# ferdean/lsa-fw

Hardware: AMD Instinct MI355X
Metric: converged eigenpairs/sec (k=20, shift-invert) (higher is better)
Workload: dtype c128

## Files before the change

### lsa-fw_amd/csrc/blas.hip

```cpp
#include "lsa_internal.h"

namespace {

constexpr int kThreads = 256;
constexpr int kColTile = 8;

template <typename T>
__device__ __forceinline__ T wave_sum(T v);
template <>
__device__ __forceinline__ double wave_sum<double>(double v) {
#pragma unroll
    for (int m = 32; m > 0; m >>= 1) v += __shfl_xor(v, m, 64);
    return v;
}
template <>
__device__ __forceinline__ cplx wave_sum<cplx>(cplx v) {
#pragma unroll
    for (int m = 32; m > 0; m >>= 1) {
        v.re += __shfl_xor(v.re, m, 64);
        v.im += __shfl_xor(v.im, m, 64);
    }
    return v;
}

// ... 775 lines not shown
                const double d = hs[j].re - s1;
                const double nu = sqrt(d < 0.0 ? 0.0 : d);
                const double inv = 1.0 / nu;
                nu_s = nu;
                c_s = s_mul(inv, s_sub(beta, s2));
            }
        }
    }
    __syncthreads();
    const double nu = nu_s, inv = 1.0 / nu;
    const cplx cc = c_s;
    if (bx == 0) {
        for (int c = threadIdx.x; c < j; c += kThreads) {
            slot[c] = first ? cplx{0.0, 0.0} : hs[c];
            if constexpr (Y) slot[lds + c] = hs[kFuseCols + c];
        }
        if (threadIdx.x == 0) {
            slot[2 * lds] = cplx{nu, 0.0};
            slot[2 * lds + 1] = cc;
        }
    }
    cplx aa = cplx{0.0, 0.0}, ab = cplx{0.0, 0.0};
    if (i < n) {
#pragma unroll
        for (int u = 0; u < 8; ++u)
            if (q + 4 * u < j) {
                if (!first) fma_acc(aa, hs[q + 4 * u], v0[u]);
                if constexpr (Y) fma_acc(ab, hs[kFuseCols + q + 4 * u], v0[u]);
            }
        for (int c = q + 32; c < j; c += 32) {
            cplx v[8];
#pragma unroll
            for (int u = 0; u < 8; ++u) v[u] = (c + 4 * u < j) ? V[i + (int64_t)(c + 4 * u) * ldv] : cplx{0.0, 0.0};
#pragma unroll
            for (int u = 0; u < 8; ++u)
                if (c + 4 * u < j) {
                    if (!first) fma_acc(aa, hs[c + 4 * u], v[u]);
                    if constexpr (Y) fma_acc(ab, hs[kFuseCols + c + 4 * u], v[u]);
                }
        }
    }
    const int l1 = (lane & 15) + 16, l2 = (lane & 15) + 32, l3 = (lane & 15) + 48;
    const cplx a1 = cplx{__shfl(aa.re, l1), __shfl(aa.im, l1)}, a2 = cplx{__shfl(aa.re, l2), __shfl(aa.im, l2)},
               a3 = cplx{__shfl(aa.re, l3), __shfl(aa.im, l3)};
    cplx b1 = cplx{0.0, 0.0}, b2 = b1, b3 = b1;
    if constexpr (Y) {
        b1 = cplx{__shfl(ab.re, l1), __shfl(ab.im, l1)};
        b2 = cplx{__shfl(ab.re, l2), __shfl(ab.im, l2)};
        b3 = cplx{__shfl(ab.re, l3), __shfl(ab.im, l3)};
    }
    double nrm = 0.0;
    if (q == 0 && i < n) {
        cplx qv = pi;
        if (!first) {
            qv = s_mul(inv, s_sub(pi, s_add(s_add(aa, a1), s_add(a2, a3))));
            V[i + (int64_t)j * ldv] = qv;
        }
        if constexpr (Y) {
            const cplx r = s_mul(inv, s_sub(s_sub(yi, s_add(s_add(ab, b1), s_add(b2, b3))), s_mul(cc, qv)));
            V[i + (int64_t)(j + 1) * ldv] = r;
            nrm = s_abs2(r);
        }
    }
    if constexpr (Y) {
        nrm = wave_sum_dpp(nrm);
        if (lane == 0) wn[wave] = nrm;
        __syncthreads();
        if (threadIdx.x == 0) nrm_part[bx] = (wn[0] + wn[1]) + (wn[2] + wn[3]);
    }
}

template <bool Y>
__global__ __launch_bounds__(kThreads) void dcgs_update_kernel(int64_t n, int j, cplx* V, int64_t ldv, const cplx* __restrict__ part, int nchunks,
                                                               int ldp, const cplx* __restrict__ y, int first, double* __restrict__ nrm_part,
                                                               cplx* __restrict__ slot, int lds, const double* __restrict__ chk_part,
                                                               double* __restrict__ chk_out) {
    dcgs_update_body<Y>((int)blockIdx.x, n, j, V, ldv, part, nchunks, ldp, y, first, nrm_part, slot, lds, chk_part, chk_out);
}

__global__ __launch_bounds__(kThreads) void dcgs_update_batch_kernel(int64_t n, int64_t ldv, int nchunks, int ldp, int lds, DcgsBatchArgs a) {
    const int z = blockIdx.z;
    dcgs_update_body<true>((int)blockIdx.x, n, a.j[z], a.V[z], ldv, a.part[z], nchunks, ldp, a.y[z], a.first[z], a.nrm_part[z], a.slot[z], lds,
                           (const double*)nullptr, (double*)nullptr);
}

__global__ __launch_bounds__(kThreads) void dcgs_norm_kernel(const double* __restrict__ nrm_part, int nparts, cplx* __restrict__ out) {
    __shared__ double smem[4];
    const double t = parts_sum(nrm_part, nparts, smem);
    if (threadIdx.x == 0) s_from(out[0], sqrt(t), 0.0);
}

__global__ __launch_bounds__(kThreads) void col_stats_kernel(int64_t n, const cplx* __restrict__ X, int64_t ldx, double* __restrict__ nrm_part,
                                                             double* __restrict__ mag_part, long long* __restrict__ idx_part) {
    __shared__ double ssum[4];
    __shared__ double smag[kThreads];
    __shared__ long long sidx[kThreads];
    const cplx* x = X + (size_t)blockIdx.y * (size_t)ldx;
    double s = 0.0, best = -1.0;
    long long bi = -1;
    const int64_t stride = (int64_t)gridDim.x * blockDim.x;
    for (int64_t i = (int64_t)blockIdx.x * blockDim.x + threadIdx.x; i < n; i += stride) {
        const double a = s_abs2(x[i]);
        s += a;
        if (a > best) {
            best = a;
            bi = i;
        }
    }
    const double tot = block_sum<double>(s, ssum);
    smag[threadIdx.x] = best;
    sidx[threadIdx.x] = bi;
    __syncthreads();
    for (int o = kThreads / 2; o > 0; o >>= 1) {
        if ((int)threadIdx.x < o) {
            const double m2 = smag[threadIdx.x + o];
            const long long i2 = sidx[threadIdx.x + o];
            if (m2 > smag[threadIdx.x] || (m2 == smag[threadIdx.x] && i2 >= 0 && (sidx[threadIdx.x] < 0 || i2 < sidx[threadIdx.x]))) {
                smag[threadIdx.x] = m2;
                sidx[threadIdx.x] = i2;
            }
        }
        __syncthreads();
    }
    if (threadIdx.x == 0) {
        const size_t at = (size_t)blockIdx.y * gridDim.x + blockIdx.x;
        nrm_part[at] = tot;
        mag_part[at] = smag[0];
        idx_part[at] = sidx[0];
    }
}

__global__ __launch_bounds__(kThreads) void col_phase_kernel(int64_t n, cplx* __restrict__ X, int64_t ldx, const double* __restrict__ nrm_part,
                                                             const double* __restrict__ mag_part, const long long* __restrict__ idx_part, int unit,
                                                             double* __restrict__ imag_part) {
    __shared__ double ssum[4];
    __shared__ double smag[kThreads];
    __shared__ long long sidx[kThreads];
    cplx* x = X + (size_t)blockIdx.y * (size_t)ldx;
    const int nb = gridDim.x;
    const size_t base = (size_t)blockIdx.y * nb;
    double s = 0.0, best = -1.0;
    long long bi = -1;
    for (int q = threadIdx.x; q < nb; q += kThreads) {
        s += nrm_part[base + q];
        const double m2 = mag_part[base + q];
        const long long i2 = idx_part[base + q];
        if (m2 > best || (m2 == best && i2 >= 0 && (bi < 0 || i2 < bi))) {
            best = m2;
            bi = i2;
        }
    }
    const double tot = block_sum<double>(s, ssum);
    smag[threadIdx.x] = best;
    sidx[threadIdx.x] = bi;
    __syncthreads();
    for (int o = kThreads / 2; o > 0; o >>= 1) {
        if ((int)threadIdx.x < o) {
            const double m2 = smag[threadIdx.x + o];
            const long long i2 = sidx[threadIdx.x + o];
            if (m2 > smag[threadIdx.x] || (m2 == smag[threadIdx.x] && i2 >= 0 && (sidx[threadIdx.x] < 0 || i2 < sidx[threadIdx.x]))) {
                smag[threadIdx.x] = m2;
                sidx[threadIdx.x] = i2;
            }
        }
        __syncthreads();
    }
// ... 451 lines not shown
    const FusedWork fw(work, 16);
    void *part1 = fw.part1, *part2 = fw.part2, *h1 = fw.h1, *h2 = fw.h2;
    double* nrm_part = fw.nrm_part;
    const dim3 dgrid(nchunks, (j + kColTile - 1) / kColTile);
    hipLaunchKernelGGL((cgs_dot_kernel<T>), dgrid, dim3(kThreads), 0, ctx->stream, n, j, rpb, (const T*)V, ldv, (const T*)y, (T*)part1, kFuseCols,
                       (const T*)nullptr, (const T*)nullptr, (double*)nullptr);
    hipLaunchKernelGGL((cgs_axpy_kernel<T>), dim3(blocks), dim3(kThreads), 0, ctx->stream, n, j, (const T*)V, ldv, (const T*)part1, nchunks, kFuseCols,
                       (const T*)y, (T*)w, (T*)h1, (double*)nullptr, (const double*)nullptr, (double*)nullptr);
    hipLaunchKernelGGL((cgs_dot_kernel<T>), dgrid, dim3(kThreads), 0, ctx->stream, n, j, rpb, (const T*)V, ldv, (const T*)w, (T*)part2, kFuseCols,
                       (const T*)nullptr, (const T*)nullptr, (double*)nullptr);
    hipLaunchKernelGGL((cgs_axpy_kernel<T>), dim3(blocks), dim3(kThreads), 0, ctx->stream, n, j, (const T*)V, ldv, (const T*)part2, nchunks, kFuseCols,
                       (const T*)w, (T*)w, (T*)h2, nrm_part, (const double*)nullptr, (double*)nullptr);
    const int tparts = k_cgs2_tail_parts(n);
    if (M->dtype == LSA_C128)
        hipLaunchKernelGGL((cgs_tail_kernel<cplx, 16>), dim3(tparts), dim3(kThreads), 0, ctx->stream, (int32_t)n, C->rp, C->ci, (const cplx*)M->val,
                           (const cplx*)C->val, (const T*)w, (const T*)y, (const double*)nrm_part, blocks, (T*)vnext, (T*)t, j, (const T*)h1, (const T*)h2,
                           (T*)hcol_dev, tail_part);
    else
        hipLaunchKernelGGL((cgs_tail_kernel<double, 16>), dim3(tparts), dim3(kThreads), 0, ctx->stream, (int32_t)n, C->rp, C->ci, (const double*)M->val,
                           (const cplx*)C->val, (const T*)w, (const T*)y, (const double*)nrm_part, blocks, (T*)vnext, (T*)t, j, (const T*)h1, (const T*)h2,
                           (T*)hcol_dev, tail_part);
    return check_launch(ctx, "cgs2_fused_tail");
}

int k_cgs2_tail_checks(lsa_ctx* ctx, int nslots, int nparts, const double* tail_parts, double* checks) {
    if (nslots <= 0) return LSA_OK;
    hipLaunchKernelGGL(cgs_tail_checks_kernel, dim3(nslots), dim3(kThreads), 0, ctx->stream, nparts, tail_parts, checks);
    return check_launch(ctx, "cgs2_tail_checks");
}

bool k_dcgs2_fits(int64_t n, int ncv) { return cgs2_fused_shape(n, ncv + 1, nullptr); }

int k_dcgs2_step(lsa_ctx* ctx, int64_t n, int j, void* V, int64_t ldv, const void* y, int first, void* slot, int lds, void* work,
                 const void* chk_b, const void* chk_z, double* chk_out) {
    int64_t rpb = 0;
    if (!cgs2_fused_shape(n, j + 1, &rpb) || j < 0 || j + 1 > lds + 1 || (first && !y))
        return lsa_set_error(ctx, LSA_ERR_ARG, "k_dcgs2_step: shape outside the fused form");
    const int nchunks = (int)((n + rpb - 1) / rpb);
    const int blocks = (int)((n + 63) / 64);
    const FusedWork fw(work, 16);
    cplx* part = (cplx*)fw.part1;
    double *chk_part = fw.chk_part, *nrm_part = fw.nrm_part;
    const dim3 dgrid(nchunks, (j + 1 + kColTile - 1) / kColTile);
    const int ldp = 2 * kFuseCols;
    if (y) {
        hipLaunchKernelGGL((dcgs_dot_kernel<true>), dgrid, dim3(kThreads), 0, ctx->stream, n, j + 1, rpb, (const cplx*)V, ldv, (const cplx*)y, part, ldp,
                           (const cplx*)chk_b, (const cplx*)chk_z, chk_out ? chk_part : (double*)nullptr);
        hipLaunchKernelGGL((dcgs_update_kernel<true>), dim3(blocks), dim3(kThreads), 0, ctx->stream, n, j, (cplx*)V, ldv, (const cplx*)part, nchunks, ldp,
                           (const cplx*)y, first, nrm_part, (cplx*)slot, lds, (const double*)chk_part, chk_out);
    } else {
        hipLaunchKernelGGL((dcgs_dot_kernel<false>), dgrid, dim3(kThreads), 0, ctx->stream, n, j + 1, rpb, (const cplx*)V, ldv, (const cplx*)nullptr, part,
                           ldp, (const cplx*)nullptr, (const cplx*)nullptr, (double*)nullptr);
        hipLaunchKernelGGL((dcgs_update_kernel<false>), dim3(blocks), dim3(kThreads), 0, ctx->stream, n, j, (cplx*)V, ldv, (const cplx*)part, nchunks, ldp,
                           (const cplx*)nullptr, 0, (double*)nullptr, (cplx*)slot, lds, (const double*)nullptr, (double*)nullptr);
    }
    return check_launch(ctx, "dcgs2_step");
}

int k_dcgs2_norm(lsa_ctx* ctx, int64_t n, void* work, void* slot, int lds) {
    double* nrm_part = FusedWork(work, 16).nrm_part;
    hipLaunchKernelGGL(dcgs_norm_kernel, dim3(1), dim3(kThreads), 0, ctx->stream, (const double*)nrm_part, (int)((n + 63) / 64),
                       (cplx*)slot + 2 * (size_t)lds + 2);
    return check_launch(ctx, "dcgs2_norm");
}

int k_dcgs2_tail(lsa_ctx* ctx, int64_t n, int j, const void* V, int64_t ldv, const void* y, void* work, const lsa_mat* M, const lsa_mat* C, void* t,
                 double* tail_part, void* slot, int lds) {
    const int blocks = (int)((n + 63) / 64);
    double* nrm_part = FusedWork(work, 16).nrm_part;
    const cplx* w = (const cplx*)V + (size_t)(j + 1) * (size_t)ldv;
    cplx* nout = (cplx*)slot + 2 * (size_t)lds + 2;
    const int tparts = k_cgs2_tail_parts(n);
    if (M->dtype == LSA_C128)
        hipLaunchKernelGGL((cgs_tail_kernel<cplx, 16, true>), dim3(tparts), dim3(kThreads), 0, ctx->stream, (int32_t)n, C->rp, C->ci, (const cplx*)M->val,
                           (const cplx*)C->val, w, (const cplx*)y, (const double*)nrm_part, blocks, (cplx*)nullptr, (cplx*)t, 0, (const cplx*)nullptr,
                           (const cplx*)nullptr, nout, tail_part);
    else
        hipLaunchKernelGGL((cgs_tail_kernel<double, 16, true>), dim3(tparts), dim3(kThreads), 0, ctx->stream, (int32_t)n, C->rp, C->ci,
                           (const double*)M->val, (const cplx*)C->val, w, (const cplx*)y, (const double*)nrm_part, blocks, (cplx*)nullptr, (cplx*)t, 0,
                           (const cplx*)nullptr, (const cplx*)nullptr, nout, tail_part);
    return check_launch(ctx, "dcgs2_tail");
}

int k_dcgs2_step_batch(lsa_ctx* ctx, int J, int64_t n, const int32_t* j, void* const* V, int64_t ldv, const void* const* y, const int32_t* first,
                       void* const* slot, int lds, void* const* work) {
    if (J < 1 || J > kKrylovGroupMax) return lsa_set_error(ctx, LSA_ERR_ARG, "k_dcgs2_step_batch: J = %d outside [1, %d]", J, kKrylovGroupMax);
    int64_t rpb = 0;
    int jmax = 0;
    DcgsBatchArgs a;
    memset(&a, 0, sizeof a);
    for (int z = 0; z < J; ++z) {
        if (j[z] < 0 || j[z] + 1 > lds + 1 || !cgs2_fused_shape(n, j[z] + 1, &rpb) || !y[z])
            return lsa_set_error(ctx, LSA_ERR_ARG, "k_dcgs2_step_batch: shape outside the fused form (problem %d)", z);
        jmax = std::max(jmax, (int)j[z]);
        const FusedWork fw(work[z], 16);
        a.V[z] = (cplx*)V[z];
        a.y[z] = (const cplx*)y[z];
        a.part[z] = (cplx*)fw.part1;
        a.slot[z] = (cplx*)slot[z];
        a.nrm_part[z] = fw.nrm_part;
        a.j[z] = j[z];
        a.first[z] = first[z];
    }
    const int nchunks = (int)((n + rpb - 1) / rpb);
    const int blocks = (int)((n + 63) / 64);
    const int ldp = 2 * kFuseCols;
    hipLaunchKernelGGL(dcgs_dot_batch_kernel, dim3(nchunks, (jmax + 1 + kColTile - 1) / kColTile, J), dim3(kThreads), 0, ctx->stream, n, rpb, ldv, ldp, a);
    hipLaunchKernelGGL(dcgs_update_batch_kernel, dim3(blocks, 1, J), dim3(kThreads), 0, ctx->stream, n, ldv, nchunks, ldp, lds, a);
    return check_launch(ctx, "dcgs2_step_batch");
}

int k_dcgs2_tail_batch(lsa_ctx* ctx, int J, int64_t n, const int32_t* j, void* const* V, int64_t ldv, const void* const* y, void* const* work,
                       const lsa_mat* const* M, const lsa_mat* const* C, void* const* t, double* const* tail_part, void* const* slot, int lds) {
    if (J < 1 || J > kKrylovGroupMax) return lsa_set_error(ctx, LSA_ERR_ARG, "k_dcgs2_tail_batch: J = %d outside [1, %d]", J, kKrylovGroupMax);
    TailBatchArgs a;
    memset(&a, 0, sizeof a);
    for (int z = 0; z < J; ++z) {
        if (M[z]->dtype != M[0]->dtype) return lsa_set_error(ctx, LSA_ERR_ARG, "k_dcgs2_tail_batch: real and complex M in one round (problem %d)", z);
        a.rp[z] = C[z]->rp;
        a.ci[z] = C[z]->ci;
        a.mval[z] = M[z]->val;
        a.cval[z] = (const cplx*)C[z]->val;
        a.w[z] = (const cplx*)V[z] + (size_t)(j[z] + 1) * (size_t)ldv;
        a.y[z] = (const cplx*)y[z];
        a.nrm_part[z] = FusedWork(work[z], 16).nrm_part;
        a.t[z] = (cplx*)t[z];
        a.hout[z] = (cplx*)slot[z] + 2 * (size_t)lds + 2;
        a.chk_part[z] = tail_part[z];
    }
    const int blocks = (int)((n + 63) / 64);
    const dim3 grid(k_cgs2_tail_parts(n), 1, J);
    if (M[0]->dtype == LSA_C128) hipLaunchKernelGGL((cgs_tail_batch_kernel<cplx, 16>), grid, dim3(kThreads), 0, ctx->stream, (int32_t)n, blocks, a);
    else hipLaunchKernelGGL((cgs_tail_batch_kernel<double, 16>), grid, dim3(kThreads), 0, ctx->stream, (int32_t)n, blocks, a);
    return check_launch(ctx, "dcgs2_tail_batch");
}
```

### lsa-fw_amd/csrc/lsa_internal.h

```cpp
#pragma once

#include <hip/hip_runtime.h>

#include <algorithm>
#include <cmath>
#include <cstdarg>
#include <cstdint>
#include <cstdio>
#include <cstdlib>
#include <cstring>
#include <memory>
#include <string>
#include <vector>

#include "../../include/lsa_hip.h"

struct cplx {
    double re, im;
};
static_assert(sizeof(cplx) == 16, "complex128 layout");

__host__ __device__ inline cplx make_cplx(double r, double i) { return cplx{r, i}; }

template <typename T>
// ... 172 lines not shown
}

#define LSA_HIP_CHECK(ctx, expr)                                                                         \
    do {                                                                                                 \
        hipError_t _e = (expr);                                                                          \
        if (_e != hipSuccess)                                                                            \
            return lsa_set_error((ctx), LSA_ERR_HIP, "%s failed: %s (%s:%d)", #expr, hipGetErrorString(_e), \
                                 __FILE__, __LINE__);                                                    \
    } while (0)

#define LSA_HIP_ALLOC(ctx, expr)                                                                                    \
    do {                                                                                                            \
        hipError_t _e = (expr);                                                                                     \
        if (_e != hipSuccess) {                                                                                     \
            (void)hipGetLastError();                                                                                \
            return lsa_set_error((ctx), _e == hipErrorOutOfMemory ? LSA_ERR_OOM : LSA_ERR_HIP, "%s failed: %s (%s:%d)", #expr, \
                                 hipGetErrorString(_e), __FILE__, __LINE__);                                        \
        }                                                                                                           \
    } while (0)

#define LSA_CHECK(expr)            \
    do {                           \
        int _rc = (expr);          \
        if (_rc != LSA_OK) return _rc; \
    } while (0)

template <typename F>
int lsa_time_runs(lsa_ctx* ctx, bool warm, int iters, double* avg_ms, F&& run) {
    if (warm) LSA_CHECK(run());
    LSA_HIP_CHECK(ctx, hipEventRecord(ctx->ev0, ctx->stream));
    for (int i = 0; i < iters; ++i) LSA_CHECK(run());
    LSA_HIP_CHECK(ctx, hipEventRecord(ctx->ev1, ctx->stream));
    LSA_HIP_CHECK(ctx, hipEventSynchronize(ctx->ev1));
    float ms = 0.f;
    LSA_HIP_CHECK(ctx, hipEventElapsedTime(&ms, ctx->ev0, ctx->ev1));
    *avg_ms = (double)ms / iters;
    return LSA_OK;
}

constexpr int kKrylovGroupMax = 16;


int k_spmv(lsa_ctx* ctx, const lsa_mat* A, int xdtype, const void* x, void* y);
int k_spmv_transpose(lsa_ctx* ctx, const lsa_mat* A, int conj, int xdtype, const void* x, void* y);
int k_transpose_index(lsa_ctx* ctx, const lsa_mat* A, const TransposeIndex** out);
int k_spmv_transpose_batch(lsa_ctx* ctx, int32_t J, const lsa_mat* const* mats, int conj, int xdtype, const void* const* xs, void* const* ys);
int k_spmv_batch(lsa_ctx* ctx, int32_t J, const lsa_mat* const* mats, int xdtype, const void* const* xs, void* const* ys);
void spmv_share_extras(const lsa_mat* from, lsa_mat* to);

int k_spmm(lsa_ctx* ctx, const lsa_mat* A, int32_t ncols, const void* X, int64_t ldx, void* Y, int64_t ldy);
int k_spmm_transpose(lsa_ctx* ctx, const lsa_mat* A, int conj, int32_t ncols, const void* X, int64_t ldx, void* Y, int64_t ldy);
int k_block_gram(lsa_ctx* ctx, int64_t n, int32_t p, const void* U, int64_t ldu, int32_t q, const void* W, int64_t ldw, void* G_host);

bool dense_lu_solve(int32_t r, void* Mh, void* Ah);

int k_copy(lsa_ctx* ctx, int dtype, int64_t n, const void* x, void* y);
int k_set_zero(lsa_ctx* ctx, int dtype, int64_t n, void* x);
int k_axpy(lsa_ctx* ctx, int dtype, int64_t n, const double alpha[2], const void* x, void* y);
int k_multi_dot(lsa_ctx* ctx, int dtype, int64_t n, int j, const void* V, int64_t ldv, const void* w, void* h_dev);
int k_multi_axpy_dot(lsa_ctx* ctx, int dtype, int64_t n, int j, const void* V, int64_t ldv, const void* h1_dev, void* w, void* h2_dev);
int k_multi_axpy(lsa_ctx* ctx, int dtype, int64_t n, int j, const void* V, int64_t ldv, const void* h_dev, void* w,
                 double* nrm2_dev);
int k_columns_canonical(lsa_ctx* ctx, int64_t n, int ncols, void* X, int64_t ldx, int unit, double* imag2_dev);
int k_nrm2(lsa_ctx* ctx, int dtype, int64_t n, const void* x, double* nrm2_dev);
int k_pair_nrm2(lsa_ctx* ctx, int dtype, int64_t n, const void* x, const void* y, double* nrm2_dev);
int k_mask(lsa_ctx* ctx, int dtype, int64_t n, const double* keep_dev, void* y);
int k_residual_norms(lsa_ctx* ctx, int dtype, int64_t n, const void* b, const void* z, void* w, double* nrm2_dev);
int k_scale_by_inv_norm(lsa_ctx* ctx, int dtype, int64_t n, const void* x, const double* nrm2_dev, void* y);
int k_hess_column(lsa_ctx* ctx, int dtype, int j, const void* h1, const void* h2, const double* nrm2_dev, void* hout);
size_t k_cgs2_fused_work_bytes(lsa_ctx* ctx, int64_t n, int jmax);
int k_cgs2_fused(lsa_ctx* ctx, int dtype, int64_t n, int j, const void* V, int64_t ldv, void* w, void* vnext, void* hcol_dev, void* work,
                 const void* chk_b, const void* chk_z, double* chk_out);
bool k_cgs2_tail_fits(lsa_ctx* ctx, int64_t n, int jmax, const lsa_mat* M, const lsa_mat* C);
int k_cgs2_tail_parts(int64_t n);
int k_cgs2_fused_tail(lsa_ctx* ctx, int64_t n, int j, const void* V, int64_t ldv, const void* y, void* w, void* vnext, void* hcol_dev, void* work,
                      const lsa_mat* M, const lsa_mat* C, void* t, double* tail_part);
int k_cgs2_tail_checks(lsa_ctx* ctx, int nslots, int nparts, const double* tail_parts, double* checks);
bool k_dcgs2_fits(int64_t n, int ncv);
int k_dcgs2_step(lsa_ctx* ctx, int64_t n, int j, void* V, int64_t ldv, const void* y, int first, void* slot, int lds, void* work,
                 const void* chk_b, const void* chk_z, double* chk_out);
int k_dcgs2_norm(lsa_ctx* ctx, int64_t n, void* work, void* slot, int lds);
int k_dcgs2_tail(lsa_ctx* ctx, int64_t n, int j, const void* V, int64_t ldv, const void* y, void* work, const lsa_mat* M, const lsa_mat* C, void* t,
                 double* tail_part, void* slot, int lds);
int k_dcgs2_step_batch(lsa_ctx* ctx, int J, int64_t n, const int32_t* j, void* const* V, int64_t ldv, const void* const* y, const int32_t* first,
                       void* const* slot, int lds, void* const* work);
int k_dcgs2_tail_batch(lsa_ctx* ctx, int J, int64_t n, const int32_t* j, void* const* V, int64_t ldv, const void* const* y, void* const* work,
                       const lsa_mat* const* M, const lsa_mat* const* C, void* const* t, double* const* tail_part, void* const* slot, int lds);
int k_spmv_plain_subwave_lanes(const lsa_mat* A);
int k_basis_gemm_max_cols(int dtype);
int k_basis_gemm(lsa_ctx* ctx, int dtype, int64_t n, int m, int k, const void* V, int64_t ldv, const void* Q, int ldq,
                 void* Out, int64_t ldo);
int k_scatter_rows(lsa_ctx* ctx, int dtype, int64_t n, int ncols, const int32_t* perm, const void* In, void* Out);

int basis_upload_row_permutation(lsa_ctx* ctx, const char* who, int64_t n, const int32_t* perm, int32_t** row_perm);
int basis_times_host_matrix(lsa_ctx* ctx, int dtype, int64_t n, int m, int k, const void* V, const void* Q, int ldq, void* qdev, void* Out,
                            size_t pinned_extra);
int basis_columns_to_host(lsa_ctx* ctx, int dtype, int64_t n, int ncols, const int32_t* row_perm, const void* dev, void** xtmp, int xtmp_cols, void* host);
int direct_solve_enqueue(lsa_ctx* ctx, lsa_op* op, int dtype, const void* rhs, void* y, void* z, void* r, bool refine, double* norms,
                         int direction = -1);
void stats_book_direct_solve(lsa_stats* st, int products, bool refine, double res, double bnorm);

void krylov_arm_preapply(lsa_krylov* k, bool on);
int krylov_preapply(lsa_ctx* ctx, lsa_krylov* k, int32_t m);
int krylov_restart_queued(lsa_ctx* ctx, lsa_krylov* k, int32_t m, int32_t knew, const void* Q, int32_t ldq);

struct KrylovGroupBuf {
    int32_t J, slots, nparts;
    void* Hdev;
    double *checks, *tail_parts;
};
int krylov_group_check(lsa_ctx* ctx, int32_t J, lsa_krylov* const* ks);
int krylov_group_alloc(lsa_ctx* ctx, int32_t J, lsa_krylov* const* ks, KrylovGroupBuf* gb);
void krylov_group_free(KrylovGroupBuf* gb);
int krylov_extend_batch(lsa_ctx* ctx, KrylovGroupBuf* gb, lsa_krylov* const* ks, const uint8_t* active, const int32_t* j0, int32_t j1, void* const* Hs,
                        int32_t ldh, int32_t* breakdown, int32_t* status, std::string* errs, lsa_ks_batch_info* info);
void lsa_name_problem(lsa_ctx* ctx, int32_t z);

struct lsa_ndlu;
struct lsa_op_parts {
    int64_t n;
    const lsa_mat *Kmul, *Kfac;
    lsa_ndlu* nd;
    bool plain;
    bool shift_invert, adjoint, projected, one_rank;
    double ksp_rtol;
    double normF;
    double sigma[2];
    bool* refine;
    lsa_stats* st;
};
int lsa_op_get_parts(lsa_op* op, lsa_op_parts* out);
inline int direct_solve_verdict(double ksp_rtol, double normF, bool refine, double res, double bnorm, double xnorm, bool* backward) {
    *backward = refine && res > ksp_rtol * bnorm && normF > 0.0 && res <= 1e-12 * normF * xnorm;
    if (res <= ksp_rtol * bnorm || *backward) return 0;
    return (!refine && std::isfinite(res)) ? 1 : -1;
}
inline int direct_solve_verdict(const lsa_op_parts& P, bool refine, double res, double bnorm, double xnorm, bool* backward) {
    return direct_solve_verdict(P.ksp_rtol, P.normF, refine, res, bnorm, xnorm, backward);
}

int lanczos_create_basis(lsa_ctx* ctx, lsa_op* op, int32_t ncv, int dtype, const char* who, lsa_lanczos** out);
int lanczos_create_basis_on(lsa_ctx* ctx, lsa_op* op, const lsa_op_parts& P, int32_t ncv, int dtype, const char* who, lsa_lanczos** out);
int lanczos_shape(const lsa_lanczos* l, int64_t* n, int32_t* ncv);
void lanczos_set_inner_product(lsa_lanczos* l, const lsa_mat* Q);
int lanczos_inject(lsa_ctx* ctx, lsa_lanczos* l, int32_t j, const void* host_v);
int lanczos_restart(lsa_ctx* ctx, lsa_lanczos* l, int32_t m, int32_t knew, const double* Y, int32_t ldy);
int lanczos_ritz_vectors(lsa_ctx* ctx, lsa_lanczos* l, int32_t m, int32_t nvec, const double* Y, int32_t ldy, void* X);
void* lanczos_ritz_device(const lsa_lanczos* l);
int lanczos_ritz_to_host(lsa_ctx* ctx, lsa_lanczos* l, int32_t nvec, void* X);
const int32_t* lanczos_row_permutation(const lsa_lanczos* l);
struct lanczos_check {
    const void *b, *z;
    bool refined;
    double* xnorm2_dev;
};
struct lanczos_sums {
    double res, bnorm, xnorm;
};
struct lanczos_operator {
    void* self;
    int nchecks;
    int (*enqueue)(lsa_ctx* ctx, void* self, int32_t j, const void* rhs, void* w, void* z, void* r, lanczos_check* chk);
    int (*read_back)(lsa_ctx* ctx, void* self);
    int (*judge)(lsa_ctx* ctx, void* self, int32_t j, const lanczos_sums* sums);
};
int lanczos_set_operator(lsa_ctx* ctx, lsa_lanczos* l, const lanczos_operator* hook);
// ... 78 lines not shown
```

### lsa-fw_amd/csrc/solver.hip

```cpp
#include <algorithm>
#include <chrono>
#include <cmath>
#include <complex>

#include "ndlu_internal.h"

int ilu_check_abort(lsa_ctx* ctx, lsa_ilu* pc);

namespace {

using zc = std::complex<double>;

struct KrylovSwitches {
    bool fused;
    bool four_passes;
    bool tail;
    bool delayed;
    bool timing;
    bool preapply;
};
const KrylovSwitches& krylov_switches() {
    static const KrylovSwitches sw = [] {
        const char* passes = getenv("LSA_KRYLOV_PASSES");
        return KrylovSwitches{env_flag("LSA_KRYLOV_FUSED", true), passes && atoi(passes) == 4, env_flag("LSA_KRYLOV_TAIL", true),
                              env_flag("LSA_KRYLOV_DELAYED", true), getenv("LSA_KRYLOV_TIMING") != nullptr, env_flag("LSA_KRYLOV_PREAPPLY", true)};
    }();
    return sw;
}

struct OrthWork {
    void *h1 = nullptr, *h2 = nullptr, *hcol = nullptr;
    double* nrm2 = nullptr;
    void* fused = nullptr;
    int cap = 0;
    int ensure_fused(lsa_ctx* ctx, int64_t n) {
        if (fused) return LSA_OK;
        LSA_HIP_ALLOC(ctx, hipMalloc(&fused, k_cgs2_fused_work_bytes(ctx, n, cap)));
        return LSA_OK;
    }
    int alloc(lsa_ctx* ctx, int cap_, int dtype) {
        cap = cap_;
        const size_t b = (size_t)(cap + 2) * esize(dtype);
        LSA_HIP_CHECK(ctx, hipMalloc(&h1, b));
        LSA_HIP_CHECK(ctx, hipMalloc(&h2, b));
        LSA_HIP_CHECK(ctx, hipMalloc(&hcol, b));
        LSA_HIP_CHECK(ctx, hipMalloc((void**)&nrm2, 4 * sizeof(double)));
        return LSA_OK;
    }
    void release() {
        for (void* p : {h1, h2, hcol, (void*)nrm2, fused})
            if (p) (void)hipFree(p);
        h1 = h2 = hcol = fused = nullptr;
        nrm2 = nullptr;
    }
};

struct SolveCheck {
    const void *b, *z;
    void* r;
    double* out;
};

int orthonormalize_enqueue(lsa_ctx* ctx, int dtype, int64_t n, const void* V, int64_t ldv, int j, void* w, void* vnext, OrthWork& ow,
                           void* hcol_dev, const SolveCheck* chk = nullptr) {
    const KrylovSwitches& sw = krylov_switches();
    if (sw.fused) {
        LSA_CHECK(ow.ensure_fused(ctx, n));
        const int frc = k_cgs2_fused(ctx, dtype, n, j, V, ldv, w, vnext, hcol_dev, ow.fused, chk ? chk->b : nullptr, chk ? chk->z : nullptr,
                                     chk ? chk->out : nullptr);
        if (frc <= 0) return frc;
    }
    if (chk) LSA_CHECK(k_residual_norms(ctx, dtype, n, chk->b, chk->z, chk->r, chk->out));
    LSA_CHECK(k_multi_dot(ctx, dtype, n, j, V, ldv, w, ow.h1));
    const int arc = sw.four_passes ? 1 : k_multi_axpy_dot(ctx, dtype, n, j, V, ldv, ow.h1, w, ow.h2);
    if (arc < 0) return arc;
    if (arc > 0) {
        LSA_CHECK(k_multi_axpy(ctx, dtype, n, j, V, ldv, ow.h1, w, nullptr));
        LSA_CHECK(k_multi_dot(ctx, dtype, n, j, V, ldv, w, ow.h2));
    }
    LSA_CHECK(k_multi_axpy(ctx, dtype, n, j, V, ldv, ow.h2, w, ow.nrm2));
    LSA_CHECK(k_hess_column(ctx, dtype, j, ow.h1, ow.h2, ow.nrm2, hcol_dev));
    LSA_CHECK(k_scale_by_inv_norm(ctx, dtype, n, w, ow.nrm2, vnext));
    return LSA_OK;
}

int orthonormalize(lsa_ctx* ctx, int dtype, int64_t n, const void* V, int64_t ldv, int j, void* w, void* vnext,
                   OrthWork& ow, zc* h_host) {
    LSA_CHECK(orthonormalize_enqueue(ctx, dtype, n, V, ldv, j, w, vnext, ow, ow.hcol));
    const size_t bytes = (size_t)(j + 1) * esize(dtype);
    LSA_CHECK(lsa_ensure_scratch(ctx, 0, bytes));
    LSA_HIP_CHECK(ctx, hipMemcpyAsync(ctx->pinned, ow.hcol, bytes, hipMemcpyDeviceToHost, ctx->stream));
    LSA_HIP_CHECK(ctx, hipStreamSynchronize(ctx->stream));
    if (dtype == LSA_C128) {
        const cplx* p = (const cplx*)ctx->pinned;
        for (int c = 0; c <= j; ++c) h_host[c] = zc(p[c].re, p[c].im);
    } else {
        const double* p = (const double*)ctx->pinned;
        for (int c = 0; c <= j; ++c) h_host[c] = zc(p[c], 0.0);
    }
    return LSA_OK;
}

int device_norm(lsa_ctx* ctx, int dtype, int64_t n, const void* x, double* nrm2_dev, double* out) {
    LSA_CHECK(k_nrm2(ctx, dtype, n, x, nrm2_dev));
    LSA_CHECK(lsa_ensure_scratch(ctx, 0, sizeof(double)));
    LSA_HIP_CHECK(ctx, hipMemcpyAsync(ctx->pinned, nrm2_dev, sizeof(double), hipMemcpyDeviceToHost, ctx->stream));
    LSA_HIP_CHECK(ctx, hipStreamSynchronize(ctx->stream));
    *out = std::sqrt(*(const double*)ctx->pinned);
// ... 833 lines not shown
    }
}

int lsa_krylov_shape(const lsa_krylov* k, int64_t* n, int32_t* ncv) {
    if (!k) return LSA_ERR_ARG;
    if (n) *n = k->n;
    if (ncv) *ncv = k->ncv;
    return LSA_OK;
}

int lsa_krylov_set_row_permutation(lsa_ctx* ctx, lsa_krylov* k, const int32_t* perm) {
    if (!ctx || !k) return lsa_set_error(ctx, LSA_ERR_ARG, "lsa_krylov_set_row_permutation: null argument");
    return basis_upload_row_permutation(ctx, "lsa_krylov_set_row_permutation", k->n, perm, &k->row_perm);
}

int lsa_krylov_set_start(lsa_ctx* ctx, lsa_krylov* k, const void* host_v) {
    if (!ctx || !k || !host_v) return lsa_set_error(ctx, LSA_ERR_ARG, "lsa_krylov_set_start: null argument");
    k->pre_armed = false;
    k->drop_preapply();
    LSA_HIP_CHECK(ctx, hipMemcpyAsync(k->w, host_v, (size_t)k->n * 16, hipMemcpyHostToDevice, ctx->stream));
    double nrm = 0.0;
    LSA_CHECK(device_norm(ctx, LSA_C128, k->n, k->w, k->ow.nrm2, &nrm));
    if (!(nrm > 0.0) || !std::isfinite(nrm)) return lsa_set_error(ctx, LSA_ERR_ARG, "lsa_krylov_set_start: start vector is zero or not finite");
    LSA_CHECK(k_scale_by_inv_norm(ctx, LSA_C128, k->n, k->w, k->ow.nrm2, k->V));
    LSA_HIP_CHECK(ctx, hipStreamSynchronize(ctx->stream));
    k->pipeline = true;
    return LSA_OK;
}

int lsa_krylov_inject(lsa_ctx* ctx, lsa_krylov* k, int32_t j, const void* host_v) {
    if (!ctx || !k || !host_v) return lsa_set_error(ctx, LSA_ERR_ARG, "lsa_krylov_inject: null argument");
    if (j < 0 || j > k->ncv) return lsa_set_error(ctx, LSA_ERR_ARG, "lsa_krylov_inject: index %d out of range", j);
    if (j == 0) return lsa_krylov_set_start(ctx, k, host_v);
    k->drop_preapply();
    const size_t vb = (size_t)k->n * 16;
    LSA_HIP_CHECK(ctx, hipMemcpyAsync(k->w, host_v, vb, hipMemcpyHostToDevice, ctx->stream));
    LSA_CHECK(orthonormalize(ctx, LSA_C128, k->n, k->V, k->n, j, k->w, (char*)k->V + (size_t)j * vb, k->ow, k->hcol.data()));
    const double beta = k->hcol[j].real();
    if (!(beta > 0.0) || !std::isfinite(beta)) return lsa_set_error(ctx, LSA_ERR_ARG, "lsa_krylov_inject: vector lies in the span of the basis");
    return LSA_OK;
}

enum class Orth {
    cgs2_fused,
    cgs2_staged,
    dcgs2,
};
struct StepPlan {
    bool pipelined = false;
    Orth orth = Orth::cgs2_fused;
    bool tail = false;
};

static StepPlan step_plan(lsa_ctx* ctx, const lsa_krylov* k) {
    const KrylovSwitches& sw = krylov_switches();
    const lsa_op* op = k->op;
    StepPlan p;
    if (!sw.fused) p.orth = Orth::cgs2_staged;
    else if (sw.delayed && ctx->nranks == 1 && !op->adjoint && op->n == k->n && k_dcgs2_fits(k->n, k->ncv)) p.orth = Orth::dcgs2;
    p.pipelined = k->pipeline && (k->batch > 1 || p.orth == Orth::dcgs2) && op->Kfac && op->nd && !op->pc &&
                  !(ctx->nranks > 1 && (!op->nd_dist || ctx->host_gather));
    p.tail = p.pipelined && sw.tail && sw.fused && op->Kmul && !op->adjoint && !op->keep && !op->refine && op->n == k->n &&
             k_cgs2_tail_fits(ctx, k->n, k->ncv, op->Kmul, op->Kfac);
    return p;
}

static int krylov_enqueue_step(lsa_ctx* ctx, lsa_krylov* k, const StepPlan& plan, int32_t j, int32_t slot, bool first) {
    lsa_op* op = k->op;
    const int dtype = LSA_C128;
    const size_t vb = (size_t)k->n * 16;
    const void* vj = (char*)k->V + (size_t)j * vb;
    void* vn = (char*)k->V + (size_t)(j + 1) * vb;
    void* sl = (char*)k->Hdev + (size_t)slot * krylov_slot_bytes(k->ncv);
    double* chk = k->checks + 2 * (size_t)slot;
    const bool dcgs2 = plan.orth == Orth::dcgs2;
    if (plan.orth != Orth::cgs2_staged) LSA_CHECK(k->ow.ensure_fused(ctx, k->n));
    const bool ahead = plan.tail && dcgs2 && first && k->pre_for == j && k->pre_op == op;
    k->drop_preapply();
    if (plan.tail) {
        if (!ahead && k->t_for != j) LSA_CHECK(spmv_global(ctx, op->Kmul, dtype, vj, op->t, false));
        k->t_for = -1;
        if (!ahead) LSA_CHECK(pc_global(ctx, pc_of(op), op->Kfac->row0, op->n, dtype, op->t, k->w));
        double* parts = k->tail_parts + (size_t)slot * 2 * (size_t)k->tail_nparts;
        if (dcgs2) {
            LSA_CHECK(k_dcgs2_step(ctx, k->n, j, k->V, k->n, k->w, first ? 1 : 0, sl, k->ncv, k->ow.fused, nullptr, nullptr, nullptr));
            LSA_CHECK(k_dcgs2_tail(ctx, k->n, j, k->V, k->n, k->w, k->ow.fused, op->Kmul, op->Kfac, op->t, parts, sl, k->ncv));
        } else {
            LSA_CHECK(k_cgs2_fused_tail(ctx, k->n, j + 1, k->V, k->n, k->w, k->w2, vn, sl, k->ow.fused, op->Kmul, op->Kfac, op->t, parts));
        }
        k->t_for = j + 1;
        return LSA_OK;
    }
    k->t_for = -1;
    const void* rhs = vj;
    if (op->Kmul) {
        LSA_CHECK(spmv_global(ctx, op->Kmul, dtype, vj, op->t, op->adjoint));
        rhs = op->t;
    }
    LSA_CHECK(direct_solve_enqueue(ctx, op, dtype, rhs, k->w, op->gw.z, op->gw.w, op->refine, chk));
    const SolveCheck check{rhs, op->gw.z, op->gw.w, chk};
    const bool rides = plan.orth != Orth::cgs2_staged;
    if (!rides) LSA_CHECK(k_residual_norms(ctx, dtype, op->n, check.b, check.z, check.r, check.out));
    if (op->keep) LSA_CHECK(k_mask(ctx, dtype, op->n, op->keep, k->w));
    if (dcgs2) {
        LSA_CHECK(k_dcgs2_step(ctx, k->n, j, k->V, k->n, k->w, first ? 1 : 0, sl, k->ncv, k->ow.fused, check.b, check.z, check.out));
        return k_dcgs2_norm(ctx, k->n, k->ow.fused, sl, k->ncv);
    }
    return orthonormalize_enqueue(ctx, dtype, k->n, k->V, k->n, j + 1, k->w, vn, k->ow, sl, rides ? &check : nullptr);
}

struct HessView {
    cplx* Hh;
    int32_t ldh, j0, ncv;
    cplx* col(int32_t j) const { return Hh + (size_t)j * ldh; }
};

static int judge_norm(double beta, const cplx* col, int32_t rows) {
    if (!std::isfinite(beta)) return -1;
    double colmax = 0.0;
    for (int32_t i = 0; i < rows; ++i) colmax = std::max(colmax, std::hypot(col[i].re, col[i].im));
    return beta <= 1e-14 * std::max(colmax, 1e-300) ? 1 : 0;
}

static int take_column(const HessView& H, int32_t j, const cplx* h) {
    cplx* Hj = H.col(j);
    for (int32_t i = 0; i < H.ldh; ++i) Hj[i] = i <= j + 1 ? h[i] : cplx{0.0, 0.0};
    return judge_norm(h[j + 1].re, h, j + 1);
}

static int finish_column(const HessView& H, int32_t jc, const cplx* sl) {
    cplx* Hp = H.col(jc - 1);
    const double nu = sl[2 * H.ncv].re;
    for (int32_t i = 0; i < jc; ++i) Hp[i] = cplx{Hp[i].re + sl[i].re, Hp[i].im + sl[i].im};
    Hp[jc] = cplx{nu, 0.0};
    return judge_norm(nu, Hp, jc);
}

static int provisional_column(const HessView& H, int32_t jc, const cplx* sl, bool first, cplx* h) {
    const int32_t ncv = H.ncv;
    const double inv = 1.0 / sl[2 * ncv].re;
    for (int32_t i = 0; i < jc; ++i) h[i] = sl[ncv + i];
    h[jc] = sl[2 * ncv + 1];
    if (!first) {
        for (int32_t c = 0; c < jc; ++c) {
            const cplx a = sl[c];
            const cplx* Hc = H.col(c);
            const int32_t rows = std::min(jc, std::max(H.j0, c + 1));
            for (int32_t i = 0; i <= rows; ++i) {
                h[i].re -= Hc[i].re * a.re - Hc[i].im * a.im;
                h[i].im -= Hc[i].re * a.im + Hc[i].im * a.re;
            }
        }
        for (int32_t i = 0; i <= jc; ++i) h[i] = cplx{h[i].re * inv, h[i].im * inv};
    }
    h[jc + 1] = cplx{sl[2 * ncv + 2].re, 0.0};
    return take_column(H, jc, h);
}

static int arnoldi_nonfinite(lsa_ctx* ctx, int32_t j) { return lsa_set_error(ctx, LSA_ERR_NONFINITE, "Arnoldi: non-finite norm at step %d", j); }

struct ExtendCursor {
    int32_t j;
    bool pending;
};

static int pipelined_prepare(lsa_ctx* ctx, lsa_krylov* k, const StepPlan& plan) {
    lsa_op* op = k->op;
// ... 549 lines not shown
```

Baseline: 506.3.

## Move residual check SpMV into DCGS dot kernel as extra rider blocks

Splits the old fused tail kernel in two. The C*y residual check now runs as extra blocks inside the DCGS dot-product launch, so it overlaps with the projection dots, and it no longer depends on the update. The next-vector M*w SpMV runs in a slimmer tail kernel that also folds in the norm. The aim is to shorten the critical path by doing the check work concurrently with the dots. In exchange, the two products are now read in separate passes over the sparse row structure, and the dot launch becomes heterogeneous in its block work.

```diff
diff --git a/lsa-fw_amd/csrc/blas.hip b/lsa-fw_amd/csrc/blas.hip
--- a/lsa-fw_amd/csrc/blas.hip
+++ b/lsa-fw_amd/csrc/blas.hip
@@ -881,6 +881,94 @@
     const int z = blockIdx.z;
     dcgs_update_body<true>((int)blockIdx.x, n, a.j[z], a.V[z], ldv, a.part[z], nchunks, ldp, a.y[z], a.first[z], a.nrm_part[z], a.slot[z], lds,
                            (const double*)nullptr, (double*)nullptr);
+}
+
+
+template <typename MT, int LPR, bool AM, bool AC>
+__device__ __forceinline__ void tail_rows_body(const int bx, const int nwg, int32_t n, const int32_t* __restrict__ rp, const int32_t* __restrict__ ci,
+                                               const MT* __restrict__ mval, const cplx* __restrict__ cval, const cplx* __restrict__ w,
+                                               const cplx* __restrict__ y, cplx* t, double* __restrict__ chk_part) {
+    __shared__ double csum[4][2];
+    const int64_t gid = (int64_t)bx * kThreads + threadIdx.x;
+    const int32_t lane = (int32_t)(gid % LPR);
+    const int64_t row_stride = ((int64_t)nwg * kThreads) / LPR;
+    double rw = 0.0, rb = 0.0;
+    for (int64_t row = gid / LPR; row < n; row += row_stride) {
+        const int32_t p0 = rp[row], p1 = rp[row + 1];
+        cplx am = cplx{0.0, 0.0}, ac = cplx{0.0, 0.0};
+        for (int32_t p = p0 + lane; p < p1; p += 3 * LPR) {
+            int32_t c[3];
+            MT vm[3];
+            cplx vc[3], xw[3], xy[3];
+#pragma unroll
+            for (int u = 0; u < 3; ++u) {
+                const bool in = p + u * LPR < p1;
+                c[u] = in ? ci[p + u * LPR] : 0;
+                if constexpr (AM) vm[u] = in ? mval[p + u * LPR] : scalar_traits<MT>::zero();
+                if constexpr (AC) vc[u] = in ? cval[p + u * LPR] : cplx{0.0, 0.0};
+            }
+#pragma unroll
+            for (int u = 0; u < 3; ++u) {
+                const bool in = p + u * LPR < p1;
+                if constexpr (AM) xw[u] = in ? w[c[u]] : cplx{0.0, 0.0};
+                if constexpr (AC) xy[u] = in ? y[c[u]] : cplx{0.0, 0.0};
+            }
+#pragma unroll
+            for (int u = 0; u < 3; ++u)
+                if (p + u * LPR < p1) {
+                    if constexpr (AM) fma_acc(am, vm[u], xw[u]);
+                    if constexpr (AC) fma_acc(ac, vc[u], xy[u]);
+                }
+        }
+#pragma unroll
+        for (int m = LPR / 2; m > 0; m >>= 1) {
+            if constexpr (AM) am = s_add(am, cplx{__shfl_xor(am.re, m, 64), __shfl_xor(am.im, m, 64)});
+            if constexpr (AC) ac = s_add(ac, cplx{__shfl_xor(ac.re, m, 64), __shfl_xor(ac.im, m, 64)});
+        }
+        if (lane == 0) {
+            if constexpr (AC) {
+                const cplx told = t[row];
+                rw += s_abs2(s_sub(told, ac));
+                rb += s_abs2(told);
+            }
+            if constexpr (AM) t[row] = am;
+        }
+    }
+    if constexpr (AC) {
+        rw = wave_sum_dpp(rw);
+        rb = wave_sum_dpp(rb);
+        const int wave = threadIdx.x >> 6;
+        if ((threadIdx.x & 63) == 0) {
+            csum[wave][0] = rw;
+            csum[wave][1] = rb;
+        }
+        __syncthreads();
+        if (threadIdx.x < 2) chk_part[2 * bx + threadIdx.x] = (csum[0][threadIdx.x] + csum[1][threadIdx.x]) + (csum[2][threadIdx.x] + csum[3][threadIdx.x]);
+    }
+}
+
+__global__ __launch_bounds__(kThreads) void dcgs_dot_check_kernel(int64_t n, int jc, int64_t rows_per_block, const cplx* __restrict__ V, int64_t ldv,
+                                                                  const cplx* __restrict__ y, cplx* __restrict__ part, int ldp, int nchunks, int ndot,
+                                                                  int nchk, const int32_t* __restrict__ rp, const int32_t* __restrict__ ci,
+                                                                  const cplx* __restrict__ cval, const cplx* t, double* __restrict__ chk_part) {
+    const int b = (int)blockIdx.x;
+    if (b < ndot)
+        dcgs_dot_body<true>(b % nchunks, b / nchunks, n, jc, rows_per_block, V, ldv, y, part, ldp, (const cplx*)nullptr, (const cplx*)nullptr,
+                            (double*)nullptr);
+    else
+        tail_rows_body<cplx, 16, false, true>(b - ndot, nchk, (int32_t)n, rp, ci, (const cplx*)nullptr, cval, (const cplx*)nullptr, y, (cplx*)t, chk_part);
+}
+
+template <typename MT>
+__global__ __launch_bounds__(kThreads) void cgs_tail_mw_kernel(int32_t n, const int32_t* __restrict__ rp, const int32_t* __restrict__ ci,
+                                                               const MT* __restrict__ mval, const cplx* __restrict__ w,
+                                                               const double* __restrict__ nrm_part, int nparts, cplx* t, cplx* __restrict__ hout) {
+    __shared__ double smem[4];
+    if (blockIdx.x == 0) {
+        const double tsum = parts_sum(nrm_part, nparts, smem);
+        if (threadIdx.x == 0) s_from(hout[0], sqrt(tsum), 0.0);
+    }
+    tail_rows_body<MT, 16, true, false>((int)blockIdx.x, (int)gridDim.x, n, rp, ci, mval, (const cplx*)nullptr, w, (const cplx*)nullptr, t, (double*)nullptr);
 }
 
 __global__ __launch_bounds__(kThreads) void dcgs_norm_kernel(const double* __restrict__ nrm_part, int nparts, cplx* __restrict__ out) {
@@ -1498,6 +1586,41 @@
     return check_launch(ctx, "dcgs2_tail");
 }
 
+int k_dcgs2_step_check(lsa_ctx* ctx, int64_t n, int j, void* V, int64_t ldv, const void* y, int first, void* slot, int lds, void* work,
+                       const lsa_mat* C, const void* t, double* tail_part) {
+    int64_t rpb = 0;
+    if (!cgs2_fused_shape(n, j + 1, &rpb) || j < 0 || j + 1 > lds + 1 || !y || !C)
+        return lsa_set_error(ctx, LSA_ERR_ARG, "k_dcgs2_step_check: shape outside the fused form");
+    const int nchunks = (int)((n + rpb - 1) / rpb);
+    const int blocks = (int)((n + 63) / 64);
+    const FusedWork fw(work, 16);
+    cplx* part = (cplx*)fw.part1;
+    const int ldp = 2 * kFuseCols;
+    const int ndot = nchunks * ((j + 1 + kColTile - 1) / kColTile);
+    const int nchk = k_cgs2_tail_parts(n);
+    hipLaunchKernelGGL(dcgs_dot_check_kernel, dim3(ndot + nchk), dim3(kThreads), 0, ctx->stream, n, j + 1, rpb, (const cplx*)V, ldv, (const cplx*)y, part,
+                       ldp, nchunks, ndot, nchk, C->rp, C->ci, (const cplx*)C->val, (const cplx*)t, tail_part);
+    hipLaunchKernelGGL((dcgs_update_kernel<true>), dim3(blocks), dim3(kThreads), 0, ctx->stream, n, j, (cplx*)V, ldv, (const cplx*)part, nchunks, ldp,
+                       (const cplx*)y, first, fw.nrm_part, (cplx*)slot, lds, (const double*)fw.chk_part, (double*)nullptr);
+    return check_launch(ctx, "dcgs2_step_check");
+}
+
+int k_dcgs2_tail_mw(lsa_ctx* ctx, int64_t n, int j, const void* V, int64_t ldv, void* work, const lsa_mat* M, const lsa_mat* C, void* t, void* slot,
+                    int lds) {
+    const int blocks = (int)((n + 63) / 64);
+    const double* nrm_part = FusedWork(work, 16).nrm_part;
+    const cplx* w = (const cplx*)V + (size_t)(j + 1) * (size_t)ldv;
+    cplx* nout = (cplx*)slot + 2 * (size_t)lds + 2;
+    const dim3 grid(k_cgs2_tail_parts(n));
+    if (M->dtype == LSA_C128)
+        hipLaunchKernelGGL((cgs_tail_mw_kernel<cplx>), grid, dim3(kThreads), 0, ctx->stream, (int32_t)n, C->rp, C->ci, (const cplx*)M->val, w, nrm_part,
+                           blocks, (cplx*)t, nout);
+    else
+        hipLaunchKernelGGL((cgs_tail_mw_kernel<double>), grid, dim3(kThreads), 0, ctx->stream, (int32_t)n, C->rp, C->ci, (const double*)M->val, w, nrm_part,
+                           blocks, (cplx*)t, nout);
+    return check_launch(ctx, "dcgs2_tail_mw");
+}
+
 int k_dcgs2_step_batch(lsa_ctx* ctx, int J, int64_t n, const int32_t* j, void* const* V, int64_t ldv, const void* const* y, const int32_t* first,
                        void* const* slot, int lds, void* const* work) {
     if (J < 1 || J > kKrylovGroupMax) return lsa_set_error(ctx, LSA_ERR_ARG, "k_dcgs2_step_batch: J = %d outside [1, %d]", J, kKrylovGroupMax);
diff --git a/lsa-fw_amd/csrc/lsa_internal.h b/lsa-fw_amd/csrc/lsa_internal.h
--- a/lsa-fw_amd/csrc/lsa_internal.h
+++ b/lsa-fw_amd/csrc/lsa_internal.h
@@ -278,6 +278,10 @@
 int k_dcgs2_norm(lsa_ctx* ctx, int64_t n, void* work, void* slot, int lds);
 int k_dcgs2_tail(lsa_ctx* ctx, int64_t n, int j, const void* V, int64_t ldv, const void* y, void* work, const lsa_mat* M, const lsa_mat* C, void* t,
                  double* tail_part, void* slot, int lds);
+int k_dcgs2_step_check(lsa_ctx* ctx, int64_t n, int j, void* V, int64_t ldv, const void* y, int first, void* slot, int lds, void* work,
+                       const lsa_mat* C, const void* t, double* tail_part);
+int k_dcgs2_tail_mw(lsa_ctx* ctx, int64_t n, int j, const void* V, int64_t ldv, void* work, const lsa_mat* M, const lsa_mat* C, void* t, void* slot,
+                    int lds);
 int k_dcgs2_step_batch(lsa_ctx* ctx, int J, int64_t n, const int32_t* j, void* const* V, int64_t ldv, const void* const* y, const int32_t* first,
                        void* const* slot, int lds, void* const* work);
 int k_dcgs2_tail_batch(lsa_ctx* ctx, int J, int64_t n, const int32_t* j, void* const* V, int64_t ldv, const void* const* y, void* const* work,
diff --git a/lsa-fw_amd/csrc/solver.hip b/lsa-fw_amd/csrc/solver.hip
--- a/lsa-fw_amd/csrc/solver.hip
+++ b/lsa-fw_amd/csrc/solver.hip
@@ -18,12 +18,14 @@
     bool delayed;
     bool timing;
     bool preapply;
+    bool riders;
 };
 const KrylovSwitches& krylov_switches() {
     static const KrylovSwitches sw = [] {
         const char* passes = getenv("LSA_KRYLOV_PASSES");
         return KrylovSwitches{env_flag("LSA_KRYLOV_FUSED", true), passes && atoi(passes) == 4, env_flag("LSA_KRYLOV_TAIL", true),
-                              env_flag("LSA_KRYLOV_DELAYED", true), getenv("LSA_KRYLOV_TIMING") != nullptr, env_flag("LSA_KRYLOV_PREAPPLY", true)};
+                              env_flag("LSA_KRYLOV_DELAYED", true), getenv("LSA_KRYLOV_TIMING") != nullptr, env_flag("LSA_KRYLOV_PREAPPLY", true),
+                              env_flag("LSA_KRYLOV_RIDERS", true)};
     }();
     return sw;
 }
@@ -1023,7 +1025,10 @@
         k->t_for = -1;
         if (!ahead) LSA_CHECK(pc_global(ctx, pc_of(op), op->Kfac->row0, op->n, dtype, op->t, k->w));
         double* parts = k->tail_parts + (size_t)slot * 2 * (size_t)k->tail_nparts;
-        if (dcgs2) {
+        if (dcgs2 && krylov_switches().riders) {
+            LSA_CHECK(k_dcgs2_step_check(ctx, k->n, j, k->V, k->n, k->w, first ? 1 : 0, sl, k->ncv, k->ow.fused, op->Kfac, op->t, parts));
+            LSA_CHECK(k_dcgs2_tail_mw(ctx, k->n, j, k->V, k->n, k->ow.fused, op->Kmul, op->Kfac, op->t, sl, k->ncv));
+        } else if (dcgs2) {
             LSA_CHECK(k_dcgs2_step(ctx, k->n, j, k->V, k->n, k->w, first ? 1 : 0, sl, k->ncv, k->ow.fused, nullptr, nullptr, nullptr));
             LSA_CHECK(k_dcgs2_tail(ctx, k->n, j, k->V, k->n, k->w, k->ow.fused, op->Kmul, op->Kfac, op->t, parts, sl, k->ncv));
         } else {
```

Result: no change. 515.2 (median of 6 runs) (+1.8%).
